# victordeleau/MUI-DeepAutoEncoder

Measured on AMD Instinct MI355X. Metric: training samples/sec at 3x512-dim input, batch 8192, higher is better.
Workload: dtype bf16; 1 GPU; embedding.yaml topology: 3 slots x 512 (io 1536), z=io, 4+4 layers -> 10 x Linear(1536,1536); batch 8192 rows per GPU, Adam lr 1e-5 wd 1e-4 clip 1.0, slot-blanking k=1; global_batch=8192, parallelism=dp1

## Files before the change

mui-deepautoencoder_amd/csrc/codae_common.h:

```cpp
#pragma once
#include <hip/hip_runtime.h>
#include <math.h>
#include <stdint.h>
#include <stdio.h>
#include <type_traits>

#include "codae_hip.h"

namespace codae {

void set_error(const char* fmt, ...);

#define CODAE_HIP_CHECK(expr)                                                              \
    do {                                                                                   \
        hipError_t e_ = (expr);                                                            \
        if (e_ != hipSuccess) {                                                            \
            codae::set_error("%s failed: %s (%s:%d)", #expr, hipGetErrorString(e_), __FILE__, __LINE__); \
            return CODAE_E_HIP;                                                            \
        }                                                                                  \
    } while (0)

#define CODAE_LAUNCH_CHECK()                                                               \
    do {                                                                                   \
        hipError_t e_ = hipGetLastError();                                                 \
// ... 124 lines not shown
__device__ __forceinline__ uint4 philox4x32_10(uint32_t c0, uint32_t c1, uint32_t c2, uint32_t c3, uint32_t k0, uint32_t k1) {
#pragma unroll
    for (int r = 0; r < 10; ++r) {
        const uint32_t hi0 = __umulhi(0xD2511F53u, c0), lo0 = 0xD2511F53u * c0;
        const uint32_t hi1 = __umulhi(0xCD9E8D57u, c2), lo1 = 0xCD9E8D57u * c2;
        c0 = hi1 ^ c1 ^ k0; c1 = lo1; c2 = hi0 ^ c3 ^ k1; c3 = lo0;
        k0 += 0x9E3779B9u; k1 += 0xBB67AE85u;
    }
    return make_uint4(c0, c1, c2, c3);
}

struct PresArgs {
    const uint8_t* tab;
    int S, E;
};
template <int W>
__device__ __forceinline__ uint32_t present_bits(const PresArgs& p, int64_t row, const int* sl) {
    const uint8_t* __restrict__ t = p.tab + row * p.S;
    const uint32_t p0 = t[sl[0]] != 0 ? 1u : 0u;
    if (sl[W - 1] == sl[0]) return p0 ? ((1u << W) - 1u) : 0u;
    uint32_t bits = p0;
#pragma unroll
    for (int k = 1; k < W; ++k) bits |= (t[sl[k]] != 0 ? 1u : 0u) << k;
    return bits;
}
int check_presence(const uint8_t* present, int n_slots, int io, const char* who);

struct SwapArgs {
    const int32_t* pool;
    uint32_t P;
    int S, E;
    uint64_t thresh;
    uint32_t key0, key1;
    const uint8_t* pres;
};
constexpr uint32_t SWAP_STREAM = 512u;
__device__ __forceinline__ int64_t swap_source(const SwapArgs& a, uint32_t row, int slot, uint32_t step) {
    const uint4 r = philox4x32_10((uint32_t)slot, row, step, SWAP_STREAM, a.key0, a.key1);
    if (!((uint64_t)r.x < a.thresh)) return -1;
    const uint32_t j = (uint32_t)(((uint64_t)r.y * a.P) >> 32);
    const uint32_t q = a.pool ? (uint32_t)a.pool[j] : j;
    if (q == row) return -1;
    if (a.pres != nullptr && (a.pres[(int64_t)row * a.S + slot] == 0 || a.pres[(int64_t)q * a.S + slot] == 0)) return -1;
    return (int64_t)q;
}
int check_swap(const codae_swap* swap, int io, const uint8_t* present, int pres_slots, const char* who);
inline SwapArgs swap_args(const codae_noise* n, const codae_swap* sw, int io, const uint8_t* present) {
    SwapArgs a{};
    a.pool = sw->pool; a.P = (uint32_t)sw->n_pool; a.S = sw->n_slots; a.E = io / sw->n_slots;
    a.thresh = (uint64_t)floor((double)n->p0 * 4294967296.0);
    a.key0 = (uint32_t)(n->seed & 0xffffffffu); a.key1 = (uint32_t)(n->seed >> 32);
    a.pres = present;
    return a;
}

static inline int64_t round_up(int64_t x, int64_t m) { return (x + m - 1) / m * m; }

constexpr int GRID_NT = 256;
inline int grid_for(int64_t work_items) {
    int64_t b = (work_items + GRID_NT - 1) / GRID_NT;
    if (b < 1) b = 1;
    if (b > 2048) b = 2048;
    return (int)b;
}

enum { STORE_PLAIN = 0, STORE_WT = 1 };
int store_policy_for(int64_t out_bytes);

template <int POL>
struct TileStore {
    __amdgpu_buffer_rsrc_t rsrc;
    __device__ __forceinline__ explicit TileStore(void* tile_base) {
        if constexpr (POL != STORE_PLAIN) rsrc = __builtin_amdgcn_make_buffer_rsrc(tile_base, 0, 0x7fffffff, 0x00020000);
    }
    __device__ __forceinline__ void store16(void* p, uint32_t byte_off, u32x4 v) const {
        if constexpr (POL == STORE_PLAIN) *reinterpret_cast<u32x4*>(p) = v;
        else __builtin_amdgcn_raw_buffer_store_b128(v, rsrc, (int)byte_off, 0, 16);
    }
};

struct EnvToggles {
    int gemm_tile = -1;
    int wgrad_splitk = 0;
    int small_tile_max = 200;
    int small_stages = 4;
    int f32_gemm = 0;
    int group_tile = -1;
    bool side_priority_set = false; int side_priority = 0;
    bool no_wt = false, single_stream = false, tail_on_side = false, no_fused_loss = false, flat_adam = false,
         no_fused_norm = false, no_chain = false, no_deep_small = false,
         no_relu_bits = false,
         no_prefetch = false,
         no_defer_wgrad = false;
    bool no_folded_loss_finish = false;
    bool no_folded_bias_finish = false;
    bool no_dataset_image = false;
    int store_policy = -1;
};
const EnvToggles& env();
void env_reload();

struct GemmF32 {
    const float* A; int64_t a_rs, a_ks;
    const float* B; int64_t b_rs, b_ks;
    float* C; int64_t ldc;
    int M, N, K;
    const float* bias;
    int relu;
    const float* relu_src;
    int64_t ld_relu;
    float* colsum_part;
    const int* m_dev;
    int split_k;
    int act;
    float act_p[3];
};
int gemm_f32(const GemmF32& g, hipStream_t s);
int gemm_f32x3(const GemmF32& g, hipStream_t s);
bool gemm_f32x3_takes(const GemmF32& g);
inline int gemm_f32_colsum_rows(int M) { return (M + 63) / 64; }

constexpr int CODAE_GROUP_MAX = 16;
struct GemmF32Group {
    int n;
    GemmF32 g[CODAE_GROUP_MAX];
    int wg_begin[CODAE_GROUP_MAX + 1];
};
int gemm_f32x3_grouped(GemmF32Group& grp, hipStream_t s);

enum { OP_KC = 0,
       OP_KS = 1
};
struct LossFuse {
    int enabled;
    const float* data;
    const int32_t* row_idx;
    const int32_t* mask_id;
    const int32_t* mask_to_use;
    int nb_run, run;
    const uint8_t* table;
    int io;
    int B;
    float inv_n;
    double* parts;
};

struct GemmBf16 {
    const bf16_t* A; int64_t lda; int a_mode;
    const bf16_t* B; int64_t ldb; int b_mode;
    void* C; int64_t ldc; int c_f32;
    int M, N, K;
    const float* bias;
    int relu;
    const bf16_t* relu_src; int64_t ld_relu;
    float* colsum_part;
    int split_k;
    LossFuse loss;
    int : 32;
    uint8_t* relu_bits_out; const uint8_t* relu_bits; int64_t ld_bits;
    const void* prefetch; int64_t prefetch_bytes;
    int coscheduled;
    double* sumsq_slots;
    int act;
    float act_p[3];
    int store_policy;
};
bool gemm_bf16_supported(int M, int N, int K);

struct GemmTile { int bm, bn; };
constexpr GemmTile TILE_256x192{256, 192}, TILE_128x192{128, 192}, TILE_128x128{128, 128}, TILE_64x128{64, 128}, TILE_64x64{64, 64};
inline int ceil_div(int a, int b) { return (a + b - 1) / b; }
inline int tile_count(int M, int N, GemmTile t) { return ceil_div(M, t.bm) * ceil_div(N, t.bn); }

enum { BF16_ONE_BARRIER = 0,
       BF16_PIPELINED = 1
};
enum { SCHED_PINNED = 0,
       SCHED_COMPILER = 64
};
struct Bf16Plan {
    int family;
    int bm, bn;
    int stages;
    int loader;
    int epi;
    int sched;
    int act;
    int store_policy;
    int tiles_m, tiles_n;
    int64_t workgroups;
};
Bf16Plan gemm_bf16_plan(const GemmBf16& g);
bool gemm_bf16_takes_relu_bits(int M, int N);
int gemm_bf16_colsum_rows(const GemmBf16& g);
int gemm_bf16_loss_parts(const GemmBf16& g);
int gemm_bf16(const GemmBf16& g, hipStream_t s);
int gemm_bf16_pipe(const GemmBf16& g, const Bf16Plan& plan, hipStream_t s);
int choose_split_k(int N, int K, int rows);

struct GemmBf16Group {
    int n;
    GemmBf16 g[CODAE_GROUP_MAX];
    int wg_begin[CODAE_GROUP_MAX + 1];
};
int gemm_bf16_grouped(GemmBf16Group& grp, hipStream_t s);
struct BiasFold;
int gemm_bf16_pipe_grouped(GemmBf16Group& grp, hipStream_t s, const BiasFold* fold = nullptr);

constexpr int CODAE_CHAIN_MAX_WIDTH = 512;
constexpr int CODAE_CHAIN_MAX_LAYERS = 16;
constexpr int CODAE_CHAIN_MAX_BIAS = 6144;
struct ChainArgs {
    int L, rows, B;
    int width[CODAE_CHAIN_MAX_LAYERS + 1];
    uint32_t relu_flags;
    double* scalars;
    const bf16_t* W[CODAE_CHAIN_MAX_LAYERS];
    const bf16_t* Wt[CODAE_CHAIN_MAX_LAYERS];
    const float* bias[CODAE_CHAIN_MAX_LAYERS];
    bf16_t* act[CODAE_CHAIN_MAX_LAYERS];
    bf16_t* dact[CODAE_CHAIN_MAX_LAYERS];
    float* colsum_part[CODAE_CHAIN_MAX_LAYERS];
    const float* data; const int32_t* row_idx; const int32_t* mask_id; const uint8_t* mask_table;
    const int32_t* mask_to_use; int nb_run, run;
    float inv_n;
    double* loss_parts;
    int do_backward;
};
bool chain_supported(int L, const int* in, const int* out);
int chain_rows_per_workgroup();
int launch_chain_step(const ChainArgs& a, hipStream_t s);

int check_noise(const codae_noise* noise);
int launch_gather_noise(const codae_batch* b, const codae_noise* noise, int32_t step, const double* step_dev, void* out,
                        int out_bf16, hipStream_t s, int64_t out_ld = 0, const int32_t* noise_rows = nullptr, double* zero_norm = nullptr,
                        const uint8_t* present = nullptr, int n_slots = 0, const codae_swap* swap = nullptr, const float* swap_data = nullptr);
bool gather_image_takes(const codae_batch* b, const void* image, const void* out, int64_t out_ld);
int launch_gather_image(const codae_batch* b, const bf16_t* image, bf16_t* out, hipStream_t s, int64_t out_ld = 0, double* zero_norm = nullptr,
                        const uint8_t* present = nullptr, int n_slots = 0, const codae_noise* noise = nullptr, int32_t step = 0,
                        const double* step_dev = nullptr, const codae_swap* swap = nullptr);
int launch_noise_box_muller(const uint32_t* ra, const uint32_t* rb, float* rho, float* c, float* sn, int64_t n, hipStream_t s);
int launch_cast_bf16(const float* src, bf16_t* dst, int64_t n, hipStream_t s);
int launch_corrupt(const float* x, const float* mask, float* out, int64_t n, hipStream_t s);
int launch_expand_masks(const int32_t* mask_id, const uint8_t* table, const int32_t* k_of_mask, int B, int io,
                        int k_max, float* masks_out, float* fmask_out, hipStream_t s);
int launch_assemble_outfits(const void* src, int src_bf16, int64_t n_rows, int io, int n_slots, const int32_t* items, int Q,
                            const int32_t* blank, int leave_one_out, const uint8_t* present, void* out, int out_bf16, int64_t out_ld,
                            hipStream_t s);
int launch_outfit_scores(const float* data, int64_t n_rows, int io, int n_slots, const int32_t* items, int Q, const uint8_t* present,
                         const float* Y, int64_t y_ld, float* cos_out, float* sq_out, float* score, int32_t* n_present, hipStream_t s);
int auc_blocks(int M);
int launch_auc_counts(const float* pos, const uint8_t* pos_on, int P, const float* neg, const int32_t* neg_slot, const int32_t* neg_parent,
                      int M, int n_slots, void* parts_ws, int64_t* counts, hipStream_t s);
struct LossLaunch {
    const codae_batch* batch; const codae_noise* noise; int32_t step; const double* step_dev;
    const codae_emphasis* emph; const uint8_t* present; int n_slots;
    const float* y; void* dy; int dy_bf16; int64_t dy_ld; float scale ;
    float* colsum_part; double* parts;
    const codae_swap* swap;
};
inline int64_t loss_dy_ld(const LossLaunch& ll) { return ll.dy_ld > 0 ? ll.dy_ld : (ll.batch ? ll.batch->io : 0); }
int check_loss_launch(const char* who, const LossLaunch& ll, bool needs_dy);
int launch_mse_loss(const LossLaunch& ll, int want_grad, hipStream_t s);
int mse_loss_colsum_rows(int B);
int check_emphasis(const codae_emphasis* emph);
int launch_emph_loss(const LossLaunch& ll, hipStream_t s);
int launch_finish_emph_loss(double* scalars, double inv_n, hipStream_t s, const double* parts, int n_parts);
int check_recon_loss(const codae_recon_loss* loss, int io);
int launch_recon_loss(const LossLaunch& ll, const codae_recon_loss* loss, hipStream_t s);
// ... 109 lines not shown
```

mui-deepautoencoder_amd/csrc/engine.hip:

```cpp
#include <stdarg.h>
#include <stdlib.h>
#include <string.h>

#include <cmath>
#include <vector>

#include "layer_gemm.h"
#include <dlfcn.h>
#include <rccl/rccl.h>

namespace codae {

static thread_local char g_err[512] = "";

void set_error(const char* fmt, ...) {
    va_list ap;
    va_start(ap, fmt);
    vsnprintf(g_err, sizeof(g_err), fmt, ap);
    va_end(ap);
}

static EnvToggles g_env;
static bool g_env_loaded = false;

void env_reload() {
    EnvToggles e;
    if (const char* t = getenv("CODAE_GEMM_TILE")) {
        switch (t[0]) { case 's': e.gemm_tile = 0; break; case 'q': e.gemm_tile = 3; break; case 'x': e.gemm_tile = 6; break; case 'm': e.gemm_tile = 7; break; default: break; }
    }
    if (const char* k = getenv("CODAE_WGRAD_SPLITK")) e.wgrad_splitk = atoi(k) > 0 ? atoi(k) : 0;
    if (const char* k = getenv("CODAE_GROUP_TILE")) e.group_tile = (k[0] >= '0' && k[0] <= '2') ? k[0] - '0' : -1;
    if (const char* pr = getenv("CODAE_SIDE_PRIORITY")) { e.side_priority_set = true; e.side_priority = atoi(pr); }
    e.no_wt = getenv("CODAE_NO_WT") != nullptr;
    e.single_stream = getenv("CODAE_SINGLE_STREAM") != nullptr;
    e.tail_on_side = getenv("CODAE_TAIL_ON_SIDE") != nullptr;
    e.no_fused_loss = getenv("CODAE_NO_FUSED_LOSS") != nullptr;
    e.flat_adam = getenv("CODAE_FLAT_ADAM") != nullptr;
    e.no_fused_norm = getenv("CODAE_NO_FUSED_NORM") != nullptr;
    e.no_chain = getenv("CODAE_NO_CHAIN") != nullptr;
    e.no_deep_small = getenv("CODAE_NO_DEEP_SMALL") != nullptr;
    e.no_defer_wgrad = getenv("CODAE_NO_DEFER_WGRAD") != nullptr;
    e.no_prefetch = getenv("CODAE_NO_PREFETCH") != nullptr;
    e.no_relu_bits = getenv("CODAE_NO_RELU_BITS") != nullptr;
    e.no_folded_loss_finish = getenv("CODAE_NO_FOLDED_LOSS_FINISH") != nullptr;
    e.no_dataset_image = getenv("CODAE_NO_DATASET_IMAGE") != nullptr;
    e.no_folded_bias_finish = getenv("CODAE_NO_FOLDED_BIAS_FINISH") != nullptr;
    if (const char* k = getenv("CODAE_STORE_POLICY"))
        e.store_policy = !strcmp(k, "plain") ? STORE_PLAIN : (!strcmp(k, "wt") ? STORE_WT : -1);
    if (const char* k = getenv("CODAE_F32_GEMM")) e.f32_gemm = k[0] == 'n' ? 1 : (k[0] == 'x' ? 2 : 0);
    if (const char* k = getenv("CODAE_SMALL_TILE_MAX")) e.small_tile_max = atoi(k);
    if (const char* k = getenv("CODAE_SMALL_STAGES")) e.small_stages = atoi(k) == 2 ? 2 : 4;
    g_env = e;
    g_env_loaded = true;
}

const EnvToggles& env() {
    if (!g_env_loaded) env_reload();
    return g_env;
}

}

using namespace codae;

constexpr int CODAE_MAX_DACT = 16;

struct codae_engine {
    int L = 0;
    std::vector<int> in, out;
    std::vector<int> in_ld, out_ld;
    std::vector<uint8_t> relu;
    std::vector<uint8_t> act;
    std::vector<float> act_p;
    int max_batch = 0, max_rows = 0;
    int prec = CODAE_PREC_F32;
    std::vector<int64_t> w_off, b_off;
    int64_t n_param = 0, bias_begin = 0;
    int maxw = 0;
    std::vector<int64_t> act_off;
    int64_t act_bytes = 0, dact_one = 0, slab_bytes = 0;
    std::vector<int64_t> bits_off;
    int n_dact = 3;
    std::vector<int> split_k;
    std::vector<int64_t> part_off;
    int64_t part_floats = 0;
    int64_t loss_part_off = 0;
    int loss_part_cap = 0;
    bool chain_ok = false;
    struct PresCfg { const uint8_t* table; int64_t n_rows; int32_t n_slots; int32_t reserved; };
    struct DropCfg { float p[64]; uint64_t seed; int32_t on; int32_t reserved; };
    struct ImageCfg { const float* data; const void* image; int64_t n_rows; int32_t io; int32_t reserved; };
    struct ResCfg { uint8_t on[64]; void* ws; int64_t ws_bytes; int32_t any; int32_t reserved; };
    struct NormCfg { uint8_t on[64]; void* ws; int64_t ws_bytes; int32_t any; int32_t kind; float eps; int32_t reserved; };
    struct TrainCfg {
        codae_noise noise;
        codae_swap swap;
        codae_emphasis emph;
        int32_t emph_on, reserved;
        codae_recon_loss recon;
        codae_slot_contrast contrast;
        PresCfg pres;
        DropCfg drop;
        codae_optimizer opt;
        int32_t tied, tied_reserved;
        ImageCfg img;
        codae_weight_average avg;
        ResCfg res;
        NormCfg norm;
    } tc;
    bool recon_on() const { return tc.recon.kind != CODAE_LOSS_MSE; }
    bool contrast_on() const { return tc.contrast.weight != 0.f; }
    int n_free() const { return (L + 1) / 2; }
    std::vector<codae_tie_pair> tie_pairs;
// ... 1884 lines not shown
```

mui-deepautoencoder_amd/csrc/gemm_bf16.hip:

```cpp
#include "codae_common.h"

namespace codae {
namespace {

constexpr int BK = 64;

typedef __attribute__((address_space(3))) char lds_char;
typedef __attribute__((address_space(1))) const void gvoid;

__device__ __forceinline__ void glds16(const void* gsrc, lds_char* dst_wave_base) {
    __builtin_amdgcn_global_load_lds((gvoid*)gsrc, (__attribute__((address_space(3))) void*)dst_wave_base, 16, 0, 0);
}

template <int R>
__device__ __forceinline__ int ks_to_lds_block(int block, int kr) {
    if constexpr (R == 192) {
        const int b = block + ((kr >> 1) & 1) + 2 * ((kr >> 3) & 1);
        return b >= 12 ? b - 12 : b;
    } else if constexpr (R == 64) {
        return block ^ (((kr >> 1) & 1) | (((kr >> 3) & 1) << 1));
    } else {
        static_assert(R == 128 || R == 256, "KS image: 64, 128, 192 or 256 columns");
        return block ^ ((kr & 3) | (((kr >> 3) & 1) << 2));
    }
// ... 484 lines not shown
constexpr int BIG_TILE_MIN_WGS = 160;

}

int gemm_bf16_grouped(GemmBf16Group& grp, hipStream_t s) {
    CODAE_REQUIRE(grp.n >= 1 && grp.n <= CODAE_GROUP_MAX, "gemm_bf16_grouped: %d GEMMs", grp.n);
    auto count = [&](GemmTile t) {
        int total = 0;
        for (int j = 0; j < grp.n; ++j) {
            const GemmBf16& g = grp.g[j];
            grp.wg_begin[j] = total;
            total += tile_count(g.M, g.N, t) * g.split_k;
        }
        grp.wg_begin[grp.n] = total;
        return total;
    };
    for (int j = 0; j < grp.n; ++j) {
        const GemmBf16& g = grp.g[j];
        CODAE_REQUIRE(g.a_mode == OP_KS && g.b_mode == OP_KS && g.c_f32 && g.split_k >= 1 && g.K % BK == 0 && g.K >= BK && g.M % 8 == 0 &&
                          g.N % 8 == 0 && !g.loss.enabled && g.relu_src == nullptr && g.colsum_part == nullptr && g.bias == nullptr,
                      "gemm_bf16_grouped: GEMM %d is not a plain weight-gradient form", j);
    }
    int tile = env().group_tile;
    if (tile < 0) tile = count(TILE_128x128) >= 256 ? 0 : (count(TILE_64x128) >= 256 ? 1 : 2);
    if (tile == 0) { const int total = count(TILE_128x128); hipLaunchKernelGGL((gemm_bf16_grouped_kernel<128, 128>), dim3(total), dim3(256), 0, s, grp); }
    else if (tile == 1) { const int total = count(TILE_64x128); hipLaunchKernelGGL((gemm_bf16_grouped_kernel<64, 128>), dim3(total), dim3(256), 0, s, grp); }
    else { const int total = count(TILE_64x64); hipLaunchKernelGGL((gemm_bf16_grouped_kernel<64, 64>), dim3(total), dim3(256), 0, s, grp); }
    CODAE_LAUNCH_CHECK();
    return CODAE_OK;
}

int store_policy_for(int64_t out_bytes) {
    if (env().store_policy >= 0) return env().store_policy;
    return out_bytes <= ((int64_t)32 << 20) ? STORE_WT : STORE_PLAIN;
}

bool gemm_bf16_supported(int M, int N, int K) {
    return M > 0 && N >= 8 && K >= BK && (K % BK) == 0 && (N % 8) == 0;
}

Bf16Plan gemm_bf16_plan(const GemmBf16& g) {
    const EnvToggles& e = env();
    const bool loss = g.loss.enabled != 0;
    const bool fwd_form = g.a_mode == OP_KC && g.b_mode == OP_KC && !g.c_f32 && g.split_k == 1;
    const bool act = g.act != CODAE_ACT_NONE;

    const int big_auto = (int64_t)tile_count(g.M, g.N, TILE_256x192) * g.split_k >= BIG_TILE_MIN_WGS ? 6 : 0;
    int big = e.gemm_tile >= 0 ? e.gemm_tile : big_auto;
    if (big == 7 && loss) big = 6;
    if (big == 7 && !fwd_form) big = big_auto;

    const bool small64 = !e.no_deep_small && fwd_form && tile_count(g.M, g.N, TILE_128x128) <= e.small_tile_max;

    Bf16Plan p{};
    GemmTile tile;
    if (!act && (big == 3 || big == 6)) {
        tile = TILE_256x192; p.family = BF16_PIPELINED; p.loader = big == 3 ? 1 : 6;
    } else if (!act && big == 7) {
        tile = TILE_128x192; p.family = BF16_PIPELINED; p.loader = 7;
    } else if (small64) {
        tile = TILE_64x64; p.family = BF16_ONE_BARRIER;
    } else if (!act && !loss && fwd_form && !e.no_deep_small) {
        tile = TILE_128x192; p.family = BF16_PIPELINED; p.loader = 7;
    } else {
        tile = TILE_128x128; p.family = BF16_ONE_BARRIER;
    }
    p.bm = tile.bm; p.bn = tile.bn;
    p.tiles_m = ceil_div(g.M, tile.bm); p.tiles_n = ceil_div(g.N, tile.bn);
    p.workgroups = (int64_t)p.tiles_m * p.tiles_n * g.split_k;

    if (p.family == BF16_ONE_BARRIER) {
        const bool deep = g.a_mode == OP_KC && g.b_mode == OP_KC && !g.c_f32 && !loss && p.workgroups <= 256 && g.K / BK >= 6 &&
                          !e.no_deep_small && e.small_stages >= 4;
        p.stages = deep ? 4 : 2;
        p.act = act;
        p.epi = loss ? 3 : 0;
        p.store_policy = STORE_PLAIN;
        return p;
    }
    const bool bwd_epi = g.relu_src != nullptr || g.colsum_part != nullptr;
    const int policy = (g.store_policy == STORE_WT && g.ldc < ((int64_t)1 << 20)) ? STORE_WT : STORE_PLAIN;
    p.epi = loss ? 3 : (g.c_f32 ? 0 : (bwd_epi ? 2 : 1));
    p.store_policy = policy;
    if (g.coscheduled && p.epi == 2 && p.loader != 7 && g.a_mode == OP_KC && g.b_mode == OP_KC) { p.sched = SCHED_COMPILER; p.store_policy = STORE_PLAIN; }
    return p;
}

bool gemm_bf16_takes_relu_bits(int M, int N) {
    GemmBf16 probe{};
    probe.M = M; probe.N = N; probe.a_mode = OP_KC; probe.b_mode = OP_KC; probe.c_f32 = 0; probe.split_k = 1;
    return gemm_bf16_plan(probe).family == BF16_PIPELINED;
}

int gemm_bf16_colsum_rows(const GemmBf16& g) { return gemm_bf16_plan(g).tiles_m; }

int gemm_bf16_loss_parts(const GemmBf16& g) {
    const Bf16Plan p = gemm_bf16_plan(g);
    return p.tiles_m * p.tiles_n;
}

int choose_split_k(int N, int K, int rows) {
    const int kt = rows / 64;
    int s;
    if (kt <= 4 && env().wgrad_splitk <= 0) return 1;
    if (env().wgrad_splitk > 0) {
        s = env().wgrad_splitk;
    } else {
        const int tiles_big = tile_count(N, K, TILE_256x192);
        s = (256 + tiles_big / 2) / tiles_big;
        if (s > 8) s = 8;
        if (s > kt) s = kt;
        if (s < 1) s = 1;
        if (tiles_big * s >= BIG_TILE_MIN_WGS) return s;
        const int tiles = tile_count(N, K, TILE_128x128);
        s = (512 + tiles / 2) / tiles;
        if (s > 8) s = 8;
    }
    if (s > kt) s = kt;
    if (s < 1) s = 1;
    return s;
}

static int validate(const GemmBf16& g) {
    CODAE_REQUIRE(gemm_bf16_supported(g.M, g.N, g.K), "gemm_bf16: unsupported shape M=%d N=%d K=%d (need K %% 64 == 0, N %% 8 == 0)",
                  g.M, g.N, g.K);
    CODAE_REQUIRE(g.a_mode == OP_KC || g.M % 8 == 0, "gemm_bf16: k-strided A needs M %% 8 == 0");
    CODAE_REQUIRE(g.a_mode == OP_KC || g.M >= 8, "gemm_bf16: k-strided A needs M >= 8");
    CODAE_REQUIRE((g.lda % 8) == 0 && (g.ldb % 8) == 0 && (g.ldc % 4) == 0, "gemm_bf16: leading dimensions must keep 16-byte rows");
    CODAE_REQUIRE(g.split_k >= 1 && (g.split_k == 1 || g.c_f32), "gemm_bf16: split-K needs fp32 output slabs");
    CODAE_REQUIRE((reinterpret_cast<uintptr_t>(g.A) & 15) == 0 && (reinterpret_cast<uintptr_t>(g.B) & 15) == 0 &&
                      (reinterpret_cast<uintptr_t>(g.C) & 15) == 0,
                  "gemm_bf16: operands must be 16-byte aligned");
    CODAE_REQUIRE(g.split_k <= g.K / BK, "gemm_bf16: split_k %d > k tiles %d", g.split_k, g.K / BK);
    CODAE_REQUIRE(!g.c_f32 || (g.relu_src == nullptr && g.colsum_part == nullptr), "gemm_bf16: ReLU mask / column sums need bf16 output");
    if (g.act != CODAE_ACT_NONE) {
        CODAE_REQUIRE(!g.loss.enabled && g.a_mode == OP_KC && g.split_k == 1 && g.relu_bits == nullptr && g.relu_bits_out == nullptr &&
                          !(g.c_f32 && g.b_mode == OP_KS),
                      "gemm_bf16: an activation needs the forward / data-gradient form (k-contiguous A, unsplit, no 1-bit masks, "
                      "no fused loss, k-strided B only with bf16 output)");
    }
    if (g.loss.enabled) {
        CODAE_REQUIRE(g.a_mode == OP_KC && g.b_mode == OP_KC && !g.c_f32 && g.split_k == 1 && !g.relu && !g.relu_src,
                      "gemm_bf16: fused loss only on the plain forward form");
        CODAE_REQUIRE(g.loss.data && g.loss.parts && g.loss.io == g.N && g.loss.B <= g.M && (g.N % 8) == 0,
                      "gemm_bf16: fused loss arguments");
        CODAE_REQUIRE(!(g.loss.mask_id || g.loss.mask_to_use) || ((reinterpret_cast<uintptr_t>(g.loss.table) & 7) == 0),
                      "gemm_bf16: mask table must be 8-byte aligned");
        CODAE_REQUIRE((reinterpret_cast<uintptr_t>(g.loss.data) & 15) == 0, "gemm_bf16: dataset must be 16-byte aligned");
    }
    return CODAE_OK;
}

int gemm_bf16(const GemmBf16& g, hipStream_t s) {
    if (int rc = validate(g)) return rc;
    const Bf16Plan plan = gemm_bf16_plan(g);
    CODAE_REQUIRE(plan.workgroups < (1 << 30), "gemm_bf16: grid too large");
    if (plan.family != BF16_ONE_BARRIER) return gemm_bf16_pipe(g, plan, s);
    return plan.bm == 64 ? launch_cfg<64, 64, 2, 2>(g, plan, s) : launch_cfg<128, 128, 2, 2>(g, plan, s);
}

}
```

mui-deepautoencoder_amd/csrc/gemm_bf16_pipe.hip:

```cpp
#include "codae_common.h"
#include <type_traits>

namespace codae {
namespace {

#include "gemm_bf16_halftile.h"

constexpr int PARK_BIAS_BYTES = 1024;
template <int BM, int BN, bool C_F32, int EPI>
constexpr int pipe_smem_bytes() {
    const bool park = BM == 256;
    return 2 * (BM + BN) * 128 + (EPI == 3 ? BM * 8 : 0) + (park ? PARK_BIAS_BYTES : 0) + (park && !C_F32 && (EPI == 2 || EPI == 4) ? BM * BN / 8 : 0);
}

template <int BM, int BN, int WM, int WN, int NLB, int A_MODE, int B_MODE, bool C_F32, int SCHED = SCHED_PINNED, int EPI = 0, int POL = STORE_PLAIN>
__device__ __forceinline__ void gemm_bf16_pipe_tile(const GemmBf16& g, int tiles_n, int tiles_mn, int kt_total, int wg, int nwg,
                                                    char* smem_raw) {
    static_assert(C_F32 || EPI != 0, "a bf16 output names its epilogue");
    static_assert(SCHED == SCHED_PINNED || SCHED == SCHED_COMPILER, "SCHED");
    constexpr int NW = WM * WN;
    constexpr int SM = BM / WM, SN = BN / WN;
    constexpr int AHR = BM / 2, BHR = BN / 2;
    constexpr int TMH = SM / 32, TNH = SN / 32;
    constexpr int AH = AHR * 128, BH = BHR * 128;
    constexpr int BUF = 2 * AH + 2 * BH;
    constexpr int NLA = (NLB == 4 && NW == 8) ? 4 : (((AHR / 8) % NW == 0) ? NW : 8);
    constexpr int NA = AHR / 8 / NLA, NB = BHR / 8 / NLB;
    static_assert(NLB <= NW && NLA <= NW && (AHR / 8) % NLA == 0 && (BHR / 8) % NLB == 0, "loader waves");
    static_assert(SM % 32 == 0 && SN % 32 == 0, "wave sub-tile must split into 16-wide half tiles");
    lds_char* smem = (lds_char*)smem_raw;
    constexpr bool PARK = BM == 256;
    constexpr bool PARK_BITS = PARK && !C_F32 && (EPI == 2 || EPI == 4);
    constexpr int BIAS_OFF = 2 * BUF + (EPI == 3 ? BM * 8 : 0), BITS_OFF = BIAS_OFF + PARK_BIAS_BYTES;
    static_assert(BN * 4 <= PARK_BIAS_BYTES && BN % 32 == 0, "bias slice: one 16-B piece per lane of one wave");

    const int lane = threadIdx.x & 63;
    const int w = __builtin_amdgcn_readfirstlane(threadIdx.x >> 6);
    const int wr = w / WN, wc = w % WN;

    int bid = wg;
    if (nwg > 0) {
        const int q = nwg >> 3, r = nwg & 7, xcd = bid & 7;
        bid = (xcd < r ? xcd * (q + 1) : r * (q + 1) + (xcd - r) * q) + (bid >> 3);
    }
    const int z = bid / tiles_mn;
    const int tmn = bid - z * tiles_mn;
    constexpr int TILE_GROUP_M = 4;
    const int tiles_m = tiles_mn / tiles_n;
    const int grp = tmn / (TILE_GROUP_M * tiles_n);
    const int tm0 = grp * TILE_GROUP_M;
    const int gsz = tiles_m - tm0 < TILE_GROUP_M ? tiles_m - tm0 : TILE_GROUP_M;
    const int within = tmn - grp * (TILE_GROUP_M * tiles_n);
    const int tn = within / gsz, tm = tm0 + (within - tn * gsz);
    const int i0 = tm * BM, j0 = tn * BN;
    const int kt_begin = (int)((int64_t)kt_total * z / g.split_k);
    const int kt_end = (int)((int64_t)kt_total * (z + 1) / g.split_k);
    const int nkt = kt_end - kt_begin;

    auto a_img = [&](int tile, int h) { return smem + (tile & 1) * BUF + h * AH; };
    auto b_img = [&](int tile, int h) { return smem + (tile & 1) * BUF + 2 * AH + h * BH; };
    if constexpr (EPI == 3) {
        const LossFuse& L = g.loss;
        int* rowinfo = reinterpret_cast<int*>(smem_raw + 2 * BUF);
        for (int r = threadIdx.x; r < BM; r += 64 * NW) {
            const int i = i0 + r;
            int src = -1, id = 0;
            if (i < L.B && i < g.M) {
                src = L.row_idx ? L.row_idx[i] : i;
                if (L.mask_id != nullptr) id = L.mask_id[i];
                else if (L.mask_to_use != nullptr) id = L.mask_to_use[(int64_t)src * L.nb_run + L.run];
            }
            rowinfo[2 * r] = src; rowinfo[2 * r + 1] = id;
        }
    }

    const bool has_bias = g.bias != nullptr;
    if constexpr (PARK) {
        if (has_bias && w == NW - 1) {
            int j = j0 + 4 * lane;
            j = j + 4 <= g.N ? j : g.N - 4;
            __builtin_amdgcn_global_load_lds((gvoid*)(g.bias + j), (__attribute__((address_space(3))) void*)(smem + BIAS_OFF), 16, 0, 0);
        }
    }
    if constexpr (PARK_BITS) {
        if (g.relu_bits != nullptr) {
            constexpr int DPR = BN / 32, NI = BM * DPR / 64;
            static_assert((BM * DPR) % 64 == 0, "bit tile: whole 64-lane instructions");
#pragma unroll
            for (int q0 = 0; q0 < NI; q0 += NW) {
                const int ins = q0 + w;
                if (ins < NI) {
                    const int q = ins * 64 + lane, r = q / DPR, cd = q - r * DPR;
                    const int row = i0 + r < g.M ? i0 + r : g.M - 1;
                    int off = (j0 >> 3) + 4 * cd;
                    off = off + 4 <= (int)g.ld_bits ? off : (int)g.ld_bits - 4;
                    __builtin_amdgcn_global_load_lds((gvoid*)(g.relu_bits + (int64_t)row * g.ld_bits + off),
                                                     (__attribute__((address_space(3))) void*)(smem + BITS_OFF + ins * 256), 4, 0, 0);
                }
            }
        }
    }
    auto bias4 = [&](int jl) -> float4 {
        if constexpr (PARK) {
            const f32x4 v = *reinterpret_cast<const __attribute__((address_space(3))) f32x4*>(smem + BIAS_OFF + jl * 4);
            const bool ok = has_bias && j0 + jl < g.N;
            return make_float4(ok ? v[0] : 0.f, ok ? v[1] : 0.f, ok ? v[2] : 0.f, ok ? v[3] : 0.f);
        } else {
            return load_bias4(g.bias, g.A, j0 + jl, g.N);
        }
    };

    f32x4 acc[2][TMH][2][TNH];
#pragma unroll
    for (int a = 0; a < 2; ++a)
#pragma unroll
        for (int b = 0; b < TMH; ++b)
#pragma unroll
            for (int c = 0; c < 2; ++c)
#pragma unroll
                for (int d = 0; d < TNH; ++d) acc[a][b][c][d] = (f32x4){0.f, 0.f, 0.f, 0.f};

    auto k_loop = [&](auto al_tag, auto bl_tag) {
    constexpr bool a_loader = decltype(al_tag)::value, b_loader = decltype(bl_tag)::value;
    uint32_t a_src[2][NA], b_src[2][NB];
#pragma unroll
    for (int h = 0; h < 2; ++h) {
#pragma unroll
        for (int it = 0; it < NA; ++it) a_src[h][it] = half_src<A_MODE, AHR, SM, NLA>(g.lda, i0, g.M, h, it, a_loader ? w : 0, lane);
#pragma unroll
        for (int it = 0; it < NB; ++it) b_src[h][it] = half_src<B_MODE, BHR, SN, NLB>(g.ldb, j0, g.N, h, it, b_loader ? w : 0, lane);
    }
    const int64_t a_step = (A_MODE == OP_KC ? BK : (int64_t)BK * g.lda) * 2;
    const int64_t b_step = (B_MODE == OP_KC ? BK : (int64_t)BK * g.ldb) * 2;
    const char* a_base = reinterpret_cast<const char*>(g.A) + kt_begin * a_step;
    const char* b_base = reinterpret_cast<const char*>(g.B) + kt_begin * b_step;
    auto issue_a = [&](int tile, int h) {
        if constexpr (a_loader) {
            const char* base = a_base + (int64_t)(tile < nkt ? tile : nkt - 1) * a_step;
            lds_char* img = a_img(tile, h);
#pragma unroll
            for (int it = 0; it < NA; ++it) glds16(base, a_src[h][it], img + (it * NLA + w) * 1024);
        }
    };
    auto issue_b = [&](int tile, int h) {
        if constexpr (b_loader) {
            const char* base = b_base + (int64_t)(tile < nkt ? tile : nkt - 1) * b_step;
            lds_char* img = b_img(tile, h);
#pragma unroll
            for (int it = 0; it < NB; ++it) glds16(base, b_src[h][it], img + (it * NLB + w) * 1024);
        }
    };

    bf16x8 a0x[TMH][2], a0y[TMH][2], a1[TMH][2], b0[TNH][2], b1[TNH][2];

    auto read_a = [&](bf16x8 (&dst)[TMH][2], int tile, int h) {
#pragma unroll
        for (int mt = 0; mt < TMH; ++mt) dst[mt][0] = read_frag<A_MODE, AHR, 0>(a_img(tile, h), wr * TMH + mt, lane);
#pragma unroll
        for (int mt = 0; mt < TMH; ++mt) dst[mt][1] = read_frag<A_MODE, AHR, 1>(a_img(tile, h), wr * TMH + mt, lane);
    };
    auto read_b = [&](bf16x8 (&dst)[TNH][2], int tile, int h) {
#pragma unroll
        for (int nt = 0; nt < TNH; ++nt) dst[nt][0] = read_frag<B_MODE, BHR, 0>(b_img(tile, h), wc * TNH + nt, lane);
#pragma unroll
        for (int nt = 0; nt < TNH; ++nt) dst[nt][1] = read_frag<B_MODE, BHR, 1>(b_img(tile, h), wc * TNH + nt, lane);
    };
    auto mma = [&](const bf16x8 (&a)[TMH][2], const bf16x8 (&b)[TNH][2], int mh, int nh) {
#pragma unroll
        for (int s = 0; s < 2; ++s)
#pragma unroll
            for (int mt = 0; mt < TMH; ++mt)
#pragma unroll
                for (int nt = 0; nt < TNH; ++nt)
                    acc[mh][mt][nh][nt] = __builtin_amdgcn_mfma_f32_16x16x32_bf16(b[nt][s], a[mt][s], acc[mh][mt][nh][nt], 0, 0, 0);
    };
    auto wait_dma = [&](auto ca, auto cb) {
        constexpr int CA = decltype(ca)::value, CB = decltype(cb)::value;
        constexpr int N = (a_loader ? CA * NA : 0) + (b_loader ? CB * NB : 0);
        if constexpr (a_loader || b_loader) wait_vmcnt<N>();
    };
    auto wait_for_a = [&]() { wait_dma(std::integral_constant<int, 2>{}, std::integral_constant<int, 3>{}); };
    auto wait_for_b = [&]() { wait_dma(std::integral_constant<int, 3>{}, std::integral_constant<int, 2>{}); };

    issue_a(0, 0); issue_b(0, 0); issue_a(0, 1); issue_b(0, 1);
    issue_a(1, 0); issue_b(1, 0); issue_a(1, 1); issue_b(1, 1);
    wait_dma(std::integral_constant<int, 3>{}, std::integral_constant<int, 4>{});
    phase_barrier();
    read_a(a0x, 0, 0);
    wait_dma(std::integral_constant<int, 3>{}, std::integral_constant<int, 3>{});
    phase_barrier();
    read_b(b0, 0, 0);

    constexpr int KEEP_A = A_MODE == OP_KC ? 2 * TMH : 0, KEEP_B = B_MODE == OP_KC ? 2 * TNH : 0;
    auto phase_order = [&](auto nread_tag, auto ndma_tag) {
        if constexpr (A_MODE == OP_KC && B_MODE == OP_KC && SCHED == SCHED_PINNED) {
            constexpr int NREAD = decltype(nread_tag)::value, NDMA = decltype(ndma_tag)::value;
#pragma unroll
            for (int i = 0; i < 6; ++i) {
                __builtin_amdgcn_sched_group_barrier(0x008, 1, 0);
                if (i < NREAD) __builtin_amdgcn_sched_group_barrier(0x100, 1, 0);
            }
#pragma unroll
            for (int i = 0; i < 4; ++i) {
                __builtin_amdgcn_sched_group_barrier(0x008, 1, 0);
                if (i < NDMA) __builtin_amdgcn_sched_group_barrier(0x020, 1, 0);
            }
            __builtin_amdgcn_sched_group_barrier(0x008, 2, 0);
        }
    };
    constexpr bool PINP = (A_MODE == OP_KC && B_MODE == OP_KC) && SCHED == SCHED_PINNED;
    using RA = std::integral_constant<int, 2 * TMH>;
    using RB = std::integral_constant<int, 2 * TNH>;
    using DA = std::integral_constant<int, a_loader ? NA : 0>;
    using DB = std::integral_constant<int, b_loader ? NB : 0>;
    auto ktile = [&](int t, bf16x8 (&a0)[TMH][2], bf16x8 (&a0n)[TMH][2]) {
        wait_for_a();
        phase_barrier<KEEP_B, PINP>();
        if constexpr (A_MODE == OP_KS) settle(a0);
        if constexpr (B_MODE == OP_KS) settle(b0);
        issue_a(t + 2, 0);
        read_a(a1, t, 1);
        mma(a0, b0, 0, 0);
        phase_order(RA{}, DA{});
        wait_for_b();
        phase_barrier<KEEP_A, PINP>();
        if constexpr (A_MODE == OP_KS) settle(a1);
        issue_b(t + 2, 0);
        read_b(b1, t, 1);
        mma(a1, b0, 1, 0);
        phase_order(RB{}, DB{});
        wait_for_a();
        phase_barrier<KEEP_B, PINP>();
        if constexpr (B_MODE == OP_KS) settle(b1);
        issue_a(t + 2, 1);
        read_a(a0n, t + 1, 0);
        mma(a1, b1, 1, 1);
        phase_order(RA{}, DA{});
        wait_for_b();
        phase_barrier<KEEP_A, PINP>();
        issue_b(t + 2, 1);
        read_b(b0, t + 1, 0);
        mma(a0, b1, 0, 1);
        phase_order(RB{}, DB{});
    };
    int t = 0;
    for (; t + 1 < nkt; t += 2) {
        ktile(t, a0x, a0y);
        ktile(t + 1, a0y, a0x);
    }
    if (t < nkt) ktile(t, a0x, a0y);
    if constexpr (A_MODE == OP_KS || B_MODE == OP_KS) {
        asm volatile("s_waitcnt lgkmcnt(0)" ::: "memory");
        if constexpr (A_MODE == OP_KS) { settle(a0x); settle(a0y); }
        if constexpr (B_MODE == OP_KS) settle(b0);
    }
    };
    {
        const bool al = (NLA == NW) || (w < NLA), bl = (NLB == NW) || (w < NLB);
        if constexpr (NLA == NW && NLB == NW) k_loop(std::true_type{}, std::true_type{});
        else if constexpr (NLA == NW) { if (bl) k_loop(std::true_type{}, std::true_type{}); else k_loop(std::true_type{}, std::false_type{}); }
        else {
            if (al && bl) k_loop(std::true_type{}, std::true_type{});
            else if (al) k_loop(std::true_type{}, std::false_type{});
// ... 380 lines not shown
}

template <int BM, int BN, int WM, int WN, int NLB, int A_MODE, int B_MODE, bool C_F32, int SCHED = SCHED_PINNED, int EPI = 0, int POL = STORE_PLAIN>
__global__ __launch_bounds__(64 * WM * WN, (WM * WN + 3) / 4)
void gemm_bf16_pipe_kernel(GemmBf16 g, int tiles_n, int tiles_mn, int kt_total) {
    __shared__ __attribute__((aligned(16))) char smem_raw[pipe_smem_bytes<BM, BN, C_F32, EPI>()];
    gemm_bf16_pipe_tile<BM, BN, WM, WN, NLB, A_MODE, B_MODE, C_F32, SCHED, EPI, POL>(g, tiles_n, tiles_mn, kt_total, blockIdx.x, gridDim.x, smem_raw);
}

typedef const __attribute__((address_space(4))) BiasFold* FoldArgs;
__device__ __attribute__((noinline)) void grouped_bias_finish(FoldArgs f, int fb, int n_fb, char* smem_raw) {
    constexpr int NT = 256;
    const int tl = threadIdx.x & (NT - 1), half = threadIdx.x >> 8;
    if (f->loss.scalars != nullptr && fb == n_fb - 1) {
        double* lred = reinterpret_cast<double*>(smem_raw);
        double a = 0.0, b = 0.0;
        if (half == 0) {
            const double* parts = f->loss.parts;
            for (int i = tl; i < f->loss.n_parts; i += NT) { a += parts[2 * i]; b += parts[2 * i + 1]; }
            lred[tl] = a; lred[NT + tl] = b;
        }
        __syncthreads();
        for (int o = NT / 2; o > 0; o >>= 1) {
            if (half == 0 && tl < o) { lred[tl] += lred[tl + o]; lred[NT + tl] += lred[NT + tl + o]; }
            __syncthreads();
        }
        if (threadIdx.x == 0) {
            double* sc = f->loss.scalars;
            sc[CODAE_S_SQ_FULL] += lred[0];
            sc[CODAE_S_SQ_PARTIAL] += lred[NT];
            sc[CODAE_S_LAST_LOSS] = lred[0] * f->loss.inv_n;
            sc[CODAE_S_STEP_SQ] = 0.0;
        }
        return;
    }
    const int n = f->n, total = f->col_begin[n];
    const int vb = 2 * fb + half;
    const int gc = vb * NT + tl;
    float sq = 0.f;
    if (gc < total) {
        int j = 0;
        while (j + 1 < n && gc >= f->col_begin[j + 1]) ++j;
        const int c = gc - f->col_begin[j];
        const int N = f->cols[j], R = f->rows[j];
        const float* p = f->parts[j] + c;
        float s = 0.f;
        int r = 0;
        for (; r + 32 <= R; r += 32) {
            float v[32];
#pragma unroll
            for (int u = 0; u < 32; ++u) v[u] = p[(int64_t)(r + u) * N];
#pragma unroll
            for (int u = 0; u < 32; ++u) s += v[u];
        }
        for (; r + 8 <= R; r += 8) {
            float v[8];
#pragma unroll
            for (int u = 0; u < 8; ++u) v[u] = p[(int64_t)(r + u) * N];
#pragma unroll
            for (int u = 0; u < 8; ++u) s += v[u];
        }
        for (; r < R; ++r) s += p[(int64_t)r * N];
        f->out[j][c] = s;
        sq = s * s;
    }
    if (f->sumsq != nullptr) {
#pragma unroll
        for (int o = 32; o > 0; o >>= 1) sq += __shfl_xor(sq, o);
        float* red = reinterpret_cast<float*>(smem_raw);
        if ((threadIdx.x & 63) == 0) red[threadIdx.x >> 6] = sq;
        __syncthreads();
        if (tl == 0 && vb * NT < total) {
            const float bsq = red[4 * half] + red[4 * half + 1] + red[4 * half + 2] + red[4 * half + 3];
            atomicAdd(f->sumsq + (CODAE_S_GRAD_SQ_SLOTS - CODAE_S_GRAD_SQ) + (vb & (CODAE_S_N_SLOTS - 1)), (double)bsq);
        }
    }
}
inline int bias_fold_workgroups(const BiasFold& f) {
    return f.n > 0 ? ceil_div(ceil_div(f.col_begin[f.n], 256), 2) + (f.loss.scalars != nullptr ? 1 : 0) : 0;
}
constexpr size_t GROUPED_FOLD_OFFSET = (sizeof(GemmBf16Group) + alignof(BiasFold) - 1) / alignof(BiasFold) * alignof(BiasFold);
static_assert(GROUPED_FOLD_OFFSET + sizeof(BiasFold) <= 6144, "grouped launch: kernel-argument block over its budget");

template <int POL>
__global__ __launch_bounds__(512, 2) void gemm_bf16_pipe_grouped_kernel(GemmBf16Group grp, BiasFold fold_by_value) {
    constexpr int BM = 256, BN = 192;
    __shared__ __attribute__((aligned(16))) char smem_raw[pipe_smem_bytes<BM, BN, true, 0>()];
    if ((int)blockIdx.x >= grp.wg_begin[grp.n]) {
        const FoldArgs f = (FoldArgs)((const __attribute__((address_space(4))) char*)__builtin_amdgcn_kernarg_segment_ptr() + GROUPED_FOLD_OFFSET);
        grouped_bias_finish(f, (int)blockIdx.x - grp.wg_begin[grp.n], (int)gridDim.x - grp.wg_begin[grp.n], smem_raw);
        return;
    }
    const int total = grp.wg_begin[grp.n];
    int t = (int)blockIdx.x;
    {
        const int q = total >> 3, r = total & 7, xcd = t & 7;
        t = (xcd < r ? xcd * (q + 1) : r * (q + 1) + (xcd - r) * q) + (t >> 3);
    }
    int j = 0;
    while (j + 1 < grp.n && t >= grp.wg_begin[j + 1]) ++j;
    const GemmBf16& g = grp.g[j];
    const int tiles_m = (g.M + BM - 1) / BM, tiles_n = (g.N + BN - 1) / BN;
    gemm_bf16_pipe_tile<BM, BN, 4, 2, 4, OP_KS, OP_KS, true, SCHED_PINNED, 0, POL>(g, tiles_n, tiles_m * tiles_n, g.K / BK, t - grp.wg_begin[j], 0, smem_raw);
}

#define PIPE_LAUNCH(BM, BN, NLB, AM, BMODE, CF, SCHED, EP, POL)                                                                  \
    hipLaunchKernelGGL((gemm_bf16_pipe_kernel<BM, BN, 4, 2, NLB, AM, BMODE, CF, SCHED, EP, POL>), dim3((unsigned)p.workgroups), dim3(512), 0, s, g, \
                       p.tiles_n, p.tiles_m * p.tiles_n, g.K / BK)

template <int NLB>
int launch_pipe(const GemmBf16& g, const Bf16Plan& p, hipStream_t s) {
    constexpr int BM = 256, BN = 192;
#define LAUNCH(AM, BMODE, CF, EP) \
    do { if (p.store_policy == STORE_WT) PIPE_LAUNCH(BM, BN, NLB, AM, BMODE, CF, SCHED_PINNED, EP, STORE_WT); else PIPE_LAUNCH(BM, BN, NLB, AM, BMODE, CF, SCHED_PINNED, EP, STORE_PLAIN); } while (0)
#define LAUNCH_BF16(AM, BMODE) do { if (p.epi == 2) LAUNCH(AM, BMODE, false, 2); else LAUNCH(AM, BMODE, false, 1); } while (0)
    const bool bits = p.epi == 2 && g.relu_bits != nullptr;
    const bool unmasked = p.epi == 2 && g.relu_bits == nullptr && g.relu_src == nullptr;
    if (p.sched == SCHED_COMPILER) PIPE_LAUNCH(BM, BN, NLB, OP_KC, OP_KC, false, SCHED_COMPILER, 2, STORE_PLAIN);
    else if (p.epi == 3) LAUNCH(OP_KC, OP_KC, false, 3);
    else if (g.a_mode == OP_KC && g.b_mode == OP_KC) { if (g.c_f32) LAUNCH(OP_KC, OP_KC, true, 0); else if (bits) LAUNCH(OP_KC, OP_KC, false, 4); else if (unmasked) LAUNCH(OP_KC, OP_KC, false, 5); else LAUNCH_BF16(OP_KC, OP_KC); }
    else if (g.a_mode == OP_KC && g.b_mode == OP_KS) { if (g.c_f32) LAUNCH(OP_KC, OP_KS, true, 0); else if (unmasked) LAUNCH(OP_KC, OP_KS, false, 5); else LAUNCH_BF16(OP_KC, OP_KS); }
    else if (g.a_mode == OP_KS && g.b_mode == OP_KS) { if (g.c_f32) LAUNCH(OP_KS, OP_KS, true, 0); else LAUNCH_BF16(OP_KS, OP_KS); }
    else { set_error("gemm_bf16: operand mode combination not built"); return CODAE_E_UNSUPPORTED; }
#undef LAUNCH_BF16
#undef LAUNCH
    CODAE_LAUNCH_CHECK();
    return CODAE_OK;
}

int launch_pipe_mid(const GemmBf16& g, const Bf16Plan& p, hipStream_t s) {
    const bool wt = p.store_policy == STORE_WT;
    if (p.epi == 2) { if (wt) PIPE_LAUNCH(128, 192, 4, OP_KC, OP_KC, false, SCHED_PINNED, 2, STORE_WT); else PIPE_LAUNCH(128, 192, 4, OP_KC, OP_KC, false, SCHED_PINNED, 2, STORE_PLAIN); }
    else { if (wt) PIPE_LAUNCH(128, 192, 4, OP_KC, OP_KC, false, SCHED_PINNED, 1, STORE_WT); else PIPE_LAUNCH(128, 192, 4, OP_KC, OP_KC, false, SCHED_PINNED, 1, STORE_PLAIN); }
    CODAE_LAUNCH_CHECK();
    return CODAE_OK;
}

}

int gemm_bf16_pipe_grouped(GemmBf16Group& grp, hipStream_t s, const BiasFold* fold) {
    CODAE_REQUIRE(grp.n >= 1 && grp.n <= CODAE_GROUP_MAX, "gemm_bf16_pipe_grouped: %d GEMMs", grp.n);
    int total = 0;
    int64_t out_bytes = 0;
    for (int j = 0; j < grp.n; ++j) out_bytes += (int64_t)grp.g[j].M * grp.g[j].N * 4;
    bool all_wt = store_policy_for(out_bytes) == STORE_WT;
    for (int j = 0; j < grp.n; ++j) {
        const GemmBf16& g = grp.g[j];
        CODAE_REQUIRE(g.a_mode == OP_KS && g.b_mode == OP_KS && g.c_f32 && g.split_k == 1 && g.K % BK == 0 && g.K >= BK && g.M % 8 == 0 &&
                          g.N % 8 == 0 && g.M >= 8 && g.N >= 8 && !g.loss.enabled && g.relu_src == nullptr && g.colsum_part == nullptr &&
                          g.bias == nullptr && !g.relu && (g.lda % 8) == 0 && (g.ldb % 8) == 0 && (g.ldc % 4) == 0,
                      "gemm_bf16_pipe_grouped: GEMM %d is not a plain unsplit weight-gradient form", j);
        CODAE_REQUIRE((int64_t)g.K * g.lda * 2 < (int64_t)1 << 32 && (int64_t)g.K * g.ldb * 2 < (int64_t)1 << 32,
                      "gemm_bf16_pipe_grouped: operand larger than 4 GiB");
        CODAE_REQUIRE((reinterpret_cast<uintptr_t>(g.A) & 15) == 0 && (reinterpret_cast<uintptr_t>(g.B) & 15) == 0 &&
                          (reinterpret_cast<uintptr_t>(g.C) & 15) == 0, "gemm_bf16_pipe_grouped: operands must be 16-byte aligned");
        if (g.store_policy != STORE_WT || g.ldc >= ((int64_t)1 << 20)) all_wt = false;
        grp.wg_begin[j] = total;
        total += tile_count(g.M, g.N, TILE_256x192);
    }
    grp.wg_begin[grp.n] = total;
    BiasFold f{};
    if (fold != nullptr) {
        f = *fold;
        CODAE_REQUIRE(f.n >= 1 && f.n <= CODAE_GROUP_MAX && f.col_begin[f.n] > 0, "gemm_bf16_pipe_grouped: %d bias-finish jobs", f.n);
        CODAE_REQUIRE(f.loss.scalars == nullptr || (f.loss.parts != nullptr && f.loss.n_parts > 0), "gemm_bf16_pipe_grouped: bad loss block");
    }
    const int grid = total + bias_fold_workgroups(f);
    if (all_wt) hipLaunchKernelGGL(gemm_bf16_pipe_grouped_kernel<STORE_WT>, dim3(grid), dim3(512), 0, s, grp, f);
    else hipLaunchKernelGGL(gemm_bf16_pipe_grouped_kernel<STORE_PLAIN>, dim3(grid), dim3(512), 0, s, grp, f);
    CODAE_LAUNCH_CHECK();
    return CODAE_OK;
}

int gemm_bf16_pipe(const GemmBf16& g_in, const Bf16Plan& p, hipStream_t s) {
    CODAE_REQUIRE((int64_t)(g_in.a_mode == OP_KC ? g_in.M : g_in.K) * g_in.lda * 2 < (int64_t)1 << 32 &&
                      (int64_t)(g_in.b_mode == OP_KC ? g_in.N : g_in.K) * g_in.ldb * 2 < (int64_t)1 << 32,
                  "gemm_bf16: operand larger than 4 GiB");
    GemmBf16 g = g_in;
    g.store_policy = p.store_policy;
    if (p.loader == 7) return launch_pipe_mid(g, p, s);
    return p.loader == 6 ? launch_pipe<4>(g, p, s) : launch_pipe<6>(g, p, s);
}
#undef PIPE_LAUNCH

}
```

Baseline: 7.242 million samples/s.

## Add two-phase K-tile schedule for weight-gradient GEMMs with double-buffered A fragments

Adds a SCHED_TWO_PHASE main loop for the 256x192 KS/KS fp32-output weight-gradient GEMM. Each K-tile now takes two barrier phases instead of four, and the A register fragments are double-buffered across K-tiles. This becomes the default for grouped wgrad launches and matching single launches, with CODAE_WGRAD_PHASES=4 restoring the old pinned schedule. The goal is to cut barrier and wait overhead in the wgrad pipeline, at the cost of higher register pressure and a more aggressive load/compute interleave.

```diff
diff --git a/mui-deepautoencoder_amd/csrc/codae_common.h b/mui-deepautoencoder_amd/csrc/codae_common.h
--- a/mui-deepautoencoder_amd/csrc/codae_common.h
+++ b/mui-deepautoencoder_amd/csrc/codae_common.h
@@ -230,6 +230,7 @@
 struct EnvToggles {
     int gemm_tile = -1;
     int wgrad_splitk = 0;
+    int wgrad_phases = 2;
     int small_tile_max = 200;
     int small_stages = 4;
     int f32_gemm = 0;
@@ -324,7 +325,8 @@
        BF16_PIPELINED = 1
 };
 enum { SCHED_PINNED = 0,
-       SCHED_COMPILER = 64
+       SCHED_COMPILER = 64,
+       SCHED_TWO_PHASE = 2
 };
 struct Bf16Plan {
     int family;
@@ -333,6 +335,7 @@
     int loader;
     int epi;
     int sched;
+    int phases;
     int act;
     int store_policy;
     int tiles_m, tiles_n;
diff --git a/mui-deepautoencoder_amd/csrc/engine.hip b/mui-deepautoencoder_amd/csrc/engine.hip
--- a/mui-deepautoencoder_amd/csrc/engine.hip
+++ b/mui-deepautoencoder_amd/csrc/engine.hip
@@ -29,6 +29,7 @@
         switch (t[0]) { case 's': e.gemm_tile = 0; break; case 'q': e.gemm_tile = 3; break; case 'x': e.gemm_tile = 6; break; case 'm': e.gemm_tile = 7; break; default: break; }
     }
     if (const char* k = getenv("CODAE_WGRAD_SPLITK")) e.wgrad_splitk = atoi(k) > 0 ? atoi(k) : 0;
+    if (const char* k = getenv("CODAE_WGRAD_PHASES")) e.wgrad_phases = atoi(k) == 4 ? 4 : 2;
     if (const char* k = getenv("CODAE_GROUP_TILE")) e.group_tile = (k[0] >= '0' && k[0] <= '2') ? k[0] - '0' : -1;
     if (const char* pr = getenv("CODAE_SIDE_PRIORITY")) { e.side_priority_set = true; e.side_priority = atoi(pr); }
     e.no_wt = getenv("CODAE_NO_WT") != nullptr;
diff --git a/mui-deepautoencoder_amd/csrc/gemm_bf16.hip b/mui-deepautoencoder_amd/csrc/gemm_bf16.hip
--- a/mui-deepautoencoder_amd/csrc/gemm_bf16.hip
+++ b/mui-deepautoencoder_amd/csrc/gemm_bf16.hip
@@ -590,6 +590,7 @@
     const int policy = (g.store_policy == STORE_WT && g.ldc < ((int64_t)1 << 20)) ? STORE_WT : STORE_PLAIN;
     p.epi = loss ? 3 : (g.c_f32 ? 0 : (bwd_epi ? 2 : 1));
     p.store_policy = policy;
+    p.phases = (tile.bm == 256 && g.a_mode == OP_KS && g.b_mode == OP_KS && g.c_f32 && g.split_k == 1 && e.wgrad_phases != 4) ? 2 : 4;
     if (g.coscheduled && p.epi == 2 && p.loader != 7 && g.a_mode == OP_KC && g.b_mode == OP_KC) { p.sched = SCHED_COMPILER; p.store_policy = STORE_PLAIN; }
     return p;
 }
diff --git a/mui-deepautoencoder_amd/csrc/gemm_bf16_pipe.hip b/mui-deepautoencoder_amd/csrc/gemm_bf16_pipe.hip
--- a/mui-deepautoencoder_amd/csrc/gemm_bf16_pipe.hip
+++ b/mui-deepautoencoder_amd/csrc/gemm_bf16_pipe.hip
@@ -17,7 +17,8 @@
 __device__ __forceinline__ void gemm_bf16_pipe_tile(const GemmBf16& g, int tiles_n, int tiles_mn, int kt_total, int wg, int nwg,
                                                     char* smem_raw) {
     static_assert(C_F32 || EPI != 0, "a bf16 output names its epilogue");
-    static_assert(SCHED == SCHED_PINNED || SCHED == SCHED_COMPILER, "SCHED");
+    static_assert(SCHED == SCHED_PINNED || SCHED == SCHED_COMPILER || SCHED == SCHED_TWO_PHASE, "SCHED");
+    static_assert(SCHED != SCHED_TWO_PHASE || (BM == 256 && A_MODE == OP_KS && B_MODE == OP_KS && C_F32), "two phases per K-tile: weight-gradient form only");
     constexpr int NW = WM * WN;
     constexpr int SM = BM / WM, SN = BN / WN;
     constexpr int AHR = BM / 2, BHR = BN / 2;
@@ -179,6 +180,41 @@
         constexpr int N = (a_loader ? CA * NA : 0) + (b_loader ? CB * NB : 0);
         if constexpr (a_loader || b_loader) wait_vmcnt<N>();
     };
+    if constexpr (SCHED == SCHED_TWO_PHASE) {
+        bf16x8 a1y[TMH][2];
+        using C2 = std::integral_constant<int, 2>;
+        using C3 = std::integral_constant<int, 3>;
+        issue_a(0, 0); issue_a(0, 1); issue_b(0, 0); issue_b(0, 1);
+        issue_a(1, 0); issue_a(1, 1); issue_b(1, 0); issue_b(1, 1);
+        wait_dma(C2{}, C3{});
+        phase_barrier();
+        read_a(a0x, 0, 0); read_a(a1, 0, 1); read_b(b0, 0, 0);
+        auto ktile2 = [&](int t, bf16x8 (&a0)[TMH][2], bf16x8 (&a1x)[TMH][2], bf16x8 (&a0n)[TMH][2], bf16x8 (&a1n)[TMH][2]) {
+            wait_dma(C2{}, C2{});
+            phase_barrier();
+            settle(a0); settle(a1x); settle(b0);
+            issue_a(t + 2, 0); issue_a(t + 2, 1); issue_b(t + 2, 0);
+            read_b(b1, t, 1);
+            mma(a0, b0, 0, 0);
+            mma(a1x, b0, 1, 0);
+            wait_dma(C2{}, C2{});
+            phase_barrier();
+            settle(b1);
+            issue_b(t + 2, 1);
+            read_a(a0n, t + 1, 0); read_a(a1n, t + 1, 1); read_b(b0, t + 1, 0);
+            mma(a1x, b1, 1, 1);
+            mma(a0, b1, 0, 1);
+        };
+        int t = 0;
+        for (; t + 1 < nkt; t += 2) {
+            ktile2(t, a0x, a1, a0y, a1y);
+            ktile2(t + 1, a0y, a1y, a0x, a1);
+        }
+        if (t < nkt) ktile2(t, a0x, a1, a0y, a1y);
+        asm volatile("s_waitcnt lgkmcnt(0)" ::: "memory");
+        settle(a0x); settle(a0y); settle(a1); settle(a1y); settle(b0);
+        return;
+    }
     auto wait_for_a = [&]() { wait_dma(std::integral_constant<int, 2>{}, std::integral_constant<int, 3>{}); };
     auto wait_for_b = [&]() { wait_dma(std::integral_constant<int, 3>{}, std::integral_constant<int, 2>{}); };
 
@@ -725,10 +761,9 @@
 constexpr size_t GROUPED_FOLD_OFFSET = (sizeof(GemmBf16Group) + alignof(BiasFold) - 1) / alignof(BiasFold) * alignof(BiasFold);
 static_assert(GROUPED_FOLD_OFFSET + sizeof(BiasFold) <= 6144, "grouped launch: kernel-argument block over its budget");
 
-template <int POL>
-__global__ __launch_bounds__(512, 2) void gemm_bf16_pipe_grouped_kernel(GemmBf16Group grp, BiasFold fold_by_value) {
+template <int POL, int SCHED>
+__device__ __forceinline__ void grouped_tiles(const GemmBf16Group& grp, char* smem_raw) {
     constexpr int BM = 256, BN = 192;
-    __shared__ __attribute__((aligned(16))) char smem_raw[pipe_smem_bytes<BM, BN, true, 0>()];
     if ((int)blockIdx.x >= grp.wg_begin[grp.n]) {
         const FoldArgs f = (FoldArgs)((const __attribute__((address_space(4))) char*)__builtin_amdgcn_kernarg_segment_ptr() + GROUPED_FOLD_OFFSET);
         grouped_bias_finish(f, (int)blockIdx.x - grp.wg_begin[grp.n], (int)gridDim.x - grp.wg_begin[grp.n], smem_raw);
@@ -744,7 +779,17 @@
     while (j + 1 < grp.n && t >= grp.wg_begin[j + 1]) ++j;
     const GemmBf16& g = grp.g[j];
     const int tiles_m = (g.M + BM - 1) / BM, tiles_n = (g.N + BN - 1) / BN;
-    gemm_bf16_pipe_tile<BM, BN, 4, 2, 4, OP_KS, OP_KS, true, SCHED_PINNED, 0, POL>(g, tiles_n, tiles_m * tiles_n, g.K / BK, t - grp.wg_begin[j], 0, smem_raw);
+    gemm_bf16_pipe_tile<BM, BN, 4, 2, 4, OP_KS, OP_KS, true, SCHED, 0, POL>(g, tiles_n, tiles_m * tiles_n, g.K / BK, t - grp.wg_begin[j], 0, smem_raw);
+}
+template <int POL>
+__global__ __launch_bounds__(512, 2) void gemm_bf16_pipe_grouped_kernel(GemmBf16Group grp, BiasFold fold_by_value) {
+    __shared__ __attribute__((aligned(16))) char smem_raw[pipe_smem_bytes<256, 192, true, 0>()];
+    grouped_tiles<POL, SCHED_TWO_PHASE>(grp, smem_raw);
+}
+template <int POL>
+__global__ __launch_bounds__(512, 2) void gemm_bf16_pipe_wgrad4_kernel(GemmBf16Group grp, BiasFold fold_by_value) {
+    __shared__ __attribute__((aligned(16))) char smem_raw[pipe_smem_bytes<256, 192, true, 0>()];
+    grouped_tiles<POL, SCHED_PINNED>(grp, smem_raw);
 }
 
 #define PIPE_LAUNCH(BM, BN, NLB, AM, BMODE, CF, SCHED, EP, POL)                                                                  \
@@ -763,7 +808,11 @@
     else if (p.epi == 3) LAUNCH(OP_KC, OP_KC, false, 3);
     else if (g.a_mode == OP_KC && g.b_mode == OP_KC) { if (g.c_f32) LAUNCH(OP_KC, OP_KC, true, 0); else if (bits) LAUNCH(OP_KC, OP_KC, false, 4); else if (unmasked) LAUNCH(OP_KC, OP_KC, false, 5); else LAUNCH_BF16(OP_KC, OP_KC); }
     else if (g.a_mode == OP_KC && g.b_mode == OP_KS) { if (g.c_f32) LAUNCH(OP_KC, OP_KS, true, 0); else if (unmasked) LAUNCH(OP_KC, OP_KS, false, 5); else LAUNCH_BF16(OP_KC, OP_KS); }
-    else if (g.a_mode == OP_KS && g.b_mode == OP_KS) { if (g.c_f32) LAUNCH(OP_KS, OP_KS, true, 0); else LAUNCH_BF16(OP_KS, OP_KS); }
+    else if (g.a_mode == OP_KS && g.b_mode == OP_KS) {
+        if (g.c_f32 && p.phases == 2) { if (p.store_policy == STORE_WT) PIPE_LAUNCH(BM, BN, NLB, OP_KS, OP_KS, true, SCHED_TWO_PHASE, 0, STORE_WT); else PIPE_LAUNCH(BM, BN, NLB, OP_KS, OP_KS, true, SCHED_TWO_PHASE, 0, STORE_PLAIN); }
+        else if (g.c_f32) LAUNCH(OP_KS, OP_KS, true, 0);
+        else LAUNCH_BF16(OP_KS, OP_KS);
+    }
     else { set_error("gemm_bf16: operand mode combination not built"); return CODAE_E_UNSUPPORTED; }
 #undef LAUNCH_BF16
 #undef LAUNCH
@@ -809,7 +858,10 @@
         CODAE_REQUIRE(f.loss.scalars == nullptr || (f.loss.parts != nullptr && f.loss.n_parts > 0), "gemm_bf16_pipe_grouped: bad loss block");
     }
     const int grid = total + bias_fold_workgroups(f);
-    if (all_wt) hipLaunchKernelGGL(gemm_bf16_pipe_grouped_kernel<STORE_WT>, dim3(grid), dim3(512), 0, s, grp, f);
+    if (env().wgrad_phases == 4) {
+        if (all_wt) hipLaunchKernelGGL(gemm_bf16_pipe_wgrad4_kernel<STORE_WT>, dim3(grid), dim3(512), 0, s, grp, f);
+        else hipLaunchKernelGGL(gemm_bf16_pipe_wgrad4_kernel<STORE_PLAIN>, dim3(grid), dim3(512), 0, s, grp, f);
+    } else if (all_wt) hipLaunchKernelGGL(gemm_bf16_pipe_grouped_kernel<STORE_WT>, dim3(grid), dim3(512), 0, s, grp, f);
     else hipLaunchKernelGGL(gemm_bf16_pipe_grouped_kernel<STORE_PLAIN>, dim3(grid), dim3(512), 0, s, grp, f);
     CODAE_LAUNCH_CHECK();
     return CODAE_OK;
```

New measurement: 7.287 million samples/s (median of 6 runs). About the same (+0.6%).
